# image-rs/deflate-rs

Hardware: AMD Instinct MI355X
Metric: MB/s raw input encoded (Compression::Default) + compressed size vs ref (higher is better)
Workload: dtype u8; 1 GPU; enwik8 = enwik8-like synthetic text (tests/datagen.py text_like; --enwik8 PATH takes the real file): 100000000 bytes per GPU, Compression::Default, stream-exact (P1); bytes_per_gpu=100000000, level=Compression::Default, parallelism=shard1

## Files before the change

deflate-rs_amd/csrc/deflate_kernels.hip:

```cpp
#include <hip/hip_runtime.h>
#include <stdint.h>

#include <type_traits>

#ifdef MI355_MATCH_STATS
__device__ unsigned long long g_mstats[16];
__device__ unsigned long long g_sstats[16];
#define MI355_STAT_DECL uint32_t stat_[8] = {0, 0, 0, 0, 0, 0, 0, 0};
#define MI355_STAT(i, v) stat_[i] += (v);
#define MI355_STAT_FLUSH(policy)                                                          \
    for (int i_ = 0; i_ < 8; i_++) atomicAdd(&g_mstats[i_], (unsigned long long)stat_[i_]); \
    atomicMax((policy).wgmax, stat_[0]);                                                  \
    if ((threadIdx.x & 63) == 0) {                                                        \
        unsigned long long t_ = wall_clock64();                                           \
        atomicMax((policy).wgend, t_);                                                    \
        atomicAdd((policy).wgsum, t_ - (policy).t0);                                      \
    }
#endif
#include "stages.h"

namespace mi355 {

struct GBytes {
    const uint8_t* d;
// ... 203 lines not shown
}
constexpr uint32_t LINKS_PAD = 64 * 8 * LG + 64;

#ifndef MI355_MATCH_TILE
#define MI355_MATCH_TILE 21504
#endif
constexpr uint32_t MT = MI355_MATCH_TILE;
#ifndef MI355_MATCH_THREADS
#define MI355_MATCH_THREADS 1024
#endif
constexpr uint32_t MTHREADS = MI355_MATCH_THREADS;
#ifndef MI355_MATCH_U
#define MI355_MATCH_U 2
#endif
#ifndef MI355_MATCH_R
#define MI355_MATCH_R 8
#endif
#ifndef MI355_EXT_ROUNDS
#define MI355_EXT_ROUNDS 100
#endif
#ifndef MI355_EXT_DENSE
#define MI355_EXT_DENSE 1
#endif
constexpr uint32_t MCHAINS = MI355_MATCH_U;
constexpr uint32_t MW_BYTES = WINDOW_SIZE + MT + 258 + 14;
constexpr uint32_t MW_LINKS = WINDOW_SIZE + MT;

struct MatchEmit {
    uint32_t* M;
    uint32_t* Mq;
    uint64_t wstart;
    __device__ void operator()(uint32_t idx, uint32_t m, uint32_t mq) const {
        M[wstart + idx] = m;
        if (Mq) Mq[wstart + idx] = mq;
    }
};

struct TileNext {
    uint32_t* counter;
    uint32_t base, count;
    __device__ uint32_t operator()() {
        uint32_t i = atomicAdd(counter, 1u);
        return i < count ? base + i : (uint32_t)NO_POS;
    }
};
struct WavePolicy {
#ifdef MI355_MATCH_STATS
    uint32_t* wgmax;
    unsigned long long* wgend;
    unsigned long long* wgsum;
    unsigned long long t0;
#endif
    __device__ bool operator()(bool pending, bool walking, uint32_t iter) const {
        if ((iter % MI355_MATCH_R) == MI355_MATCH_R - 1) return true;
        return __builtin_amdgcn_ballot_w64(walking) == 0;
    }
    __device__ bool keep_extending(bool any, uint32_t round) const {
        uint32_t cnt = (uint32_t)__popcll(__builtin_amdgcn_ballot_w64(any));
        return cnt >= MI355_EXT_DENSE || (round < MI355_EXT_ROUNDS && cnt > 0);
    }
};

struct TileLimit {
    SegEnds sg;
    uint64_t wstart;
    uint32_t one;
    __device__ uint32_t operator()(uint32_t idx) const {
        if (sg.m == 1) return one;
        uint64_t e = seg_end(sg, wstart + idx);
        uint64_t r = e - wstart;
        return r > 0xFFFFFFFFull ? 0xFFFFFFFFu : (uint32_t)r;
    }
};

template <bool HAS_Q>
__global__ __launch_bounds__(MTHREADS) void k_match(const uint8_t* __restrict__ in, uint32_t n,
                                                    const uint16_t* __restrict__ link, uint32_t* __restrict__ M,
                                                    uint32_t* __restrict__ Mq, uint32_t checks, uint32_t checks_q,
                                                    int in_aligned4, SegEnds sg, uint32_t mt) {
    __shared__ __attribute__((aligned(16))) uint8_t s_win[MW_BYTES + 2 * MW_LINKS];
    uint8_t* const s_bytes = s_win;
    uint16_t* const s_link = reinterpret_cast<uint16_t*>(s_win + MW_BYTES);
    __shared__ uint32_t s_next;
    const uint32_t tid = threadIdx.x;
    const uint64_t E = (uint64_t)blockIdx.x * mt;
    const uint32_t wbytes = WINDOW_SIZE + mt + 258 + 14, wlinks = WINDOW_SIZE + mt;
    const uint64_t wstart = E >= WINDOW_SIZE ? E - WINDOW_SIZE : 0;
    uint32_t* sb32 = reinterpret_cast<uint32_t*>(s_bytes);
    if (in_aligned4) {
        for (uint32_t w = tid; w < wbytes / 16; w += MTHREADS) {
            uint64_t g = wstart + 16ull * w;
            uint4 v = make_uint4(0, 0, 0, 0);
            if (g + 16 <= n) {
                v = *reinterpret_cast<const uint4*>(in + g);
            } else {
                uint32_t t[4] = {0, 0, 0, 0};
                for (int b = 0; b < 16; b++)
                    if (g + b < n) t[b >> 2] |= (uint32_t)in[g + b] << (8 * (b & 3));
                v = make_uint4(t[0], t[1], t[2], t[3]);
            }
            reinterpret_cast<uint4*>(s_bytes)[w] = v;
        }
    } else {
        for (uint32_t w = tid; w < wbytes / 4; w += MTHREADS) {
            uint64_t g = wstart + 4ull * w;
            uint32_t v = 0;
            for (int b = 0; b < 4; b++)
                if (g + b < n) v |= (uint32_t)in[g + b] << (8 * b);
            sb32[w] = v;
        }
    }
    for (uint32_t w = tid; w < wlinks / 8; w += MTHREADS) {
        uint64_t g = wstart + 8ull * w;
        uint4 v = make_uint4(0, 0, 0, 0);
        if (g + 8 <= n) {
            v = *reinterpret_cast<const uint4*>(link + g);
        } else {
            uint32_t t[4] = {0, 0, 0, 0};
            for (int b = 0; b < 8; b++)
                if (g + b < n) t[b >> 1] |= (uint32_t)link[g + b] << (16 * (b & 1));
            v = make_uint4(t[0], t[1], t[2], t[3]);
        }
        uint32_t t4[4] = {v.x, v.y, v.z, v.w};
#pragma unroll
        for (int q = 0; q < 4; q++) {
            uint32_t lo = t4[q] & 0xffffu, hi = t4[q] >> 16;
            t4[q] = (lo ? lo : 0xffffu) | ((hi ? hi : 0xffffu) << 16);
        }
        reinterpret_cast<uint4*>(s_link)[w] = make_uint4(t4[0], t4[1], t4[2], t4[3]);
    }
    if (tid == 0) s_next = 0;
#ifdef MI355_MATCH_STATS
    __shared__ uint32_t s_wgmax;
    __shared__ unsigned long long s_wgend, s_wgsum;
    if (tid == 0) {
        s_wgmax = 0;
        s_wgend = 0;
        s_wgsum = 0;
    }
    const unsigned long long t_enter = wall_clock64();
#endif
    __syncthreads();
    LdsWin win{s_bytes, s_link};
    MatchEmit emit{M, HAS_Q ? Mq : nullptr, wstart};
    TileNext next{&s_next, (uint32_t)(E - wstart), mt};
#ifdef MI355_MATCH_STATS
    const unsigned long long t_start = wall_clock64();
    WavePolicy pol{&s_wgmax, &s_wgend, &s_wgsum, t_start};
#else
    WavePolicy pol;
#endif
    TileLimit lim{sg, wstart, sg.m == 1 ? (uint32_t)(sg.ends[0] - wstart) : 0u};
    match_walk_park<MCHAINS, HAS_Q>(win, next, lim, checks, checks_q, emit, pol);
#ifdef MI355_MATCH_STATS
    __syncthreads();
    if (tid == 0) {
        atomicAdd(&g_mstats[8], (unsigned long long)s_wgmax);
        atomicAdd(&g_mstats[9], 1ull);
        atomicAdd(&g_mstats[10], s_wgend - t_start);
        atomicAdd(&g_mstats[11], s_wgsum);
        atomicAdd(&g_mstats[12], t_start - t_enter);
    }
#endif
}

constexpr uint32_t BSTRIDE = WINDOW_SIZE + 8;
constexpr uint32_t SORT_CHUNK = WINDOW_SIZE / 16;

__device__ __forceinline__ uint32_t epoch_active(uint32_t n, uint64_t E) {
    const uint64_t act = n >= 2 ? (uint64_t)n - 2 : 0;
    return act > E ? (uint32_t)((act - E) < (uint64_t)WINDOW_SIZE ? (act - E) : (uint64_t)WINDOW_SIZE) : 0u;
}

__device__ __forceinline__ uint32_t block_excl_scan_1024(uint32_t v, uint32_t* red , uint32_t* total) {
    const uint32_t lane = threadIdx.x & 63, wv = threadIdx.x >> 6;
    uint32_t x = v;
#pragma unroll
    for (int off = 1; off < 64; off <<= 1) {
        uint32_t y = __shfl_up(x, off, 64);
        if (lane >= (uint32_t)off) x += y;
    }
    __syncthreads();
    if (lane == 63) red[wv] = x;
    __syncthreads();
    uint32_t add = 0, all = 0;
#pragma unroll
    for (uint32_t k = 0; k < 16; k++) {
        const uint32_t t = red[k];
        add += k < wv ? t : 0u;
        all += t;
    }
    if (total) *total = all;
    return add + x - v;
}

template <int NB>
__device__ __forceinline__ void wave_match(uint32_t d, bool valid, uint32_t* plo, uint32_t* phi) {
    const uint64_t all = __builtin_amdgcn_ballot_w64(valid);
    uint32_t lo = (uint32_t)all, hi = (uint32_t)(all >> 32);
#pragma unroll
    for (int b = 0; b < NB; b++) {
        const int32_t mine = __builtin_amdgcn_sbfe((int32_t)d, (uint32_t)b, 1u);
        const uint64_t bal = __builtin_amdgcn_ballot_w64(mine != 0);
        lo &= ~((uint32_t)bal ^ (uint32_t)mine);
        hi &= ~((uint32_t)(bal >> 32) ^ (uint32_t)mine);
    }
    *plo = lo;
    *phi = hi;
}

#ifdef MI355_MATCH_STATS
#define KS_T(i)                                                                        \
    if (threadIdx.x == 0) {                                                            \
        unsigned long long t_ = __builtin_readcyclecounter();                          \
        atomicAdd(&g_sstats[i], t_ - ks_t);                                            \
        ks_t = t_;                                                                     \
    }
#else
#define KS_T(i)
#endif
template <int NB, class Dig, class Pay, class Put>
__device__ __forceinline__ void sort_pass(uint32_t J, uint32_t* cnt , uint32_t* red, Dig dig, Pay pay, Put put,
                                          unsigned long long& ks_t, int stat0) {
    constexpr uint32_t ND = 1u << NB;
    constexpr int NBAT = SORT_CHUNK / 64;
    const uint32_t tid = threadIdx.x, lane = tid & 63, wv = tid >> 6;
    uint32_t* mine = cnt + wv * 256;
    for (uint32_t k = lane; k < 256; k += 64) mine[k] = 0;
    wave_lds_fence();
    const uint32_t cb = wv * SORT_CHUNK;
    uint32_t dc[NBAT / 4];
    uint32_t bt[NBAT / 4];
    uint32_t Jc = J;
    asm volatile("" : "+s"(Jc));
#pragma unroll
    for (int b = 0; b < NBAT; b++) {
        const uint32_t i = cb + 64 * b + lane;
        const bool valid = i < Jc;
        const uint32_t d = valid ? dig(i) : 0u;
        uint32_t plo, phi;
        wave_match<NB>(d, valid, &plo, &phi);
        const uint32_t below = __builtin_amdgcn_mbcnt_hi(phi, __builtin_amdgcn_mbcnt_lo(plo, 0u));
        const uint32_t total = (uint32_t)__builtin_popcount(plo) + (uint32_t)__builtin_popcount(phi);
        if (valid && below == 0) atomicAdd(&mine[d], total);
        if ((b & 3) == 0)
            dc[b >> 2] = d;
        else
            dc[b >> 2] |= d << (8 * (b & 3));
        const uint32_t pk = below | (below + 1 == total ? 64u : 0u) | (valid ? 128u : 0u);
        if ((b & 3) == 0)
            bt[b >> 2] = pk;
        else
            bt[b >> 2] |= pk << (8 * (b & 3));
        if ((b & 3) == 3) __builtin_amdgcn_sched_barrier(0);
    }
    __syncthreads();
    KS_T(stat0)
    uint32_t v[4] = {0, 0, 0, 0}, sum = 0;
    const uint32_t d4 = tid >> 2, w4 = (tid & 3) * 4;
    if (d4 < ND) {
#pragma unroll
        for (int k = 0; k < 4; k++) {
            v[k] = cnt[(w4 + k) * 256 + d4];
            sum += v[k];
        }
    }
    uint32_t base = block_excl_scan_1024(sum, red, nullptr);
    if (d4 < ND) {
#pragma unroll
        for (int k = 0; k < 4; k++) {
            cnt[(w4 + k) * 256 + d4] = base;
            base += v[k];
        }
    }
    __syncthreads();
    KS_T(stat0 + 1)
#pragma unroll
    for (int b = 0; b < NBAT; b++) {
        const uint32_t i = cb + 64 * b + lane;
        const uint32_t d = (dc[b >> 2] >> (8 * (b & 3))) & 0xffu;
        const uint32_t pk = (bt[b >> 2] >> (8 * (b & 3))) & 0xffu;
        const bool valid = (pk & 128u) != 0;
        const uint32_t py = valid ? pay(i) : 0u;
        const uint32_t below = pk & 63u;
        uint32_t at = 0;
        if (valid) at = mine[d];
        wave_lds_fence();
        if (valid) {
            put(at + below, py);
            if (pk & 64u) mine[d] = at + below + 1;
        }
        wave_lds_fence();
    }
    __syncthreads();
    KS_T(stat0 + 2)
}

#ifndef MI355_SORT_HOT
#define MI355_SORT_HOT 4
#endif
#ifndef MI355_SORT_ROUNDS
#define MI355_SORT_ROUNDS 1
#endif
#ifndef MI355_SORT_SB
#define MI355_SORT_SB 4
#endif
template <int NB, bool LOW, class Dig, class Pay, class Put>
__device__ __forceinline__ void sort_pass_rtn(uint32_t J, uint32_t* cnt , uint32_t* red, Dig dig, Pay pay, Put put,
                                              unsigned long long& ks_t, int stat0, bool hot_low) {
    constexpr uint32_t ND = 1u << NB;
    constexpr int NBAT = SORT_CHUNK / 64;
    const uint32_t tid = threadIdx.x, lane = tid & 63, wv = tid >> 6;
    uint32_t* mine = cnt + wv * 256;
    for (uint32_t k = lane; k < 256; k += 64) mine[k] = 0;
    wave_lds_fence();
    const uint32_t cb = wv * SORT_CHUNK;
    uint32_t dc[NBAT / 4];
    uint32_t rk[NBAT / 2];
    uint32_t Jc = J;
    asm volatile("" : "+s"(Jc));
#pragma unroll
    for (int b = 0; b < NBAT; b++) {
        const uint32_t i = cb + 64 * b + lane;
        const bool valid = i < Jc;
        const uint32_t d = valid ? dig(i) : 0u;
        const uint64_t vm = __builtin_amdgcn_ballot_w64(valid);
        uint32_t r = 0;
        uint64_t left = vm;
        bool mine_done = !valid;
#pragma unroll
        for (int round = 0; round < MI355_SORT_ROUNDS; round++) {
            if (LOW && !hot_low) break;
            if (left == 0) break;
            const uint32_t first = (uint32_t)__builtin_ctzll(left);
            const uint32_t dk = (uint32_t)__builtin_amdgcn_readlane((int)d, (int)first);
            const uint64_t mk = __builtin_amdgcn_ballot_w64(!mine_done && d == dk);
            const uint32_t nk = (uint32_t)__popcll(mk);
            if (nk < MI355_SORT_HOT) break;
            const uint32_t at = mine[dk];
            wave_lds_fence();
            const bool hot = !mine_done && d == dk;
            if (hot) r = at + __builtin_amdgcn_mbcnt_hi((uint32_t)(mk >> 32), __builtin_amdgcn_mbcnt_lo((uint32_t)mk, 0u));
            if (lane == first) mine[dk] = at + nk;
            wave_lds_fence();
            mine_done = mine_done || hot;
            left &= ~mk;
        }
        if (!mine_done) r = atomicAdd(&mine[d], 1u);
        if ((b & 3) == 0)
            dc[b >> 2] = d;
        else
            dc[b >> 2] |= d << (8 * (b & 3));
        const uint32_t pk = r | (valid ? 0x8000u : 0u);
        if ((b & 1) == 0)
            rk[b >> 1] = pk;
        else
            rk[b >> 1] |= pk << 16;
        if ((b % MI355_SORT_SB) == MI355_SORT_SB - 1) __builtin_amdgcn_sched_barrier(0);
    }
    __syncthreads();
    KS_T(stat0)
    uint32_t v[4] = {0, 0, 0, 0}, sum = 0;
    const uint32_t d4 = tid >> 2, w4 = (tid & 3) * 4;
    if (d4 < ND) {
#pragma unroll
        for (int k = 0; k < 4; k++) {
            v[k] = cnt[(w4 + k) * 256 + d4];
            sum += v[k];
        }
    }
    uint32_t base = block_excl_scan_1024(sum, red, nullptr);
    if (d4 < ND) {
#pragma unroll
        for (int k = 0; k < 4; k++) {
            cnt[(w4 + k) * 256 + d4] = base;
            base += v[k];
        }
    }
    __syncthreads();
    KS_T(stat0 + 1)
#pragma unroll
    for (int b = 0; b < NBAT; b++) {
        const uint32_t i = cb + 64 * b + lane;
        const uint32_t d = (dc[b >> 2] >> (8 * (b & 3))) & 0xffu;
        const uint32_t pk = (rk[b >> 1] >> (16 * (b & 1))) & 0xffffu;
        if (pk & 0x8000u) put(mine[d] + (pk & 0x7fffu), pay(i));
    }
    __syncthreads();
    KS_T(stat0 + 2)
}

__global__ __launch_bounds__(1024) void k_lds_order_test(uint32_t rounds, uint32_t* bad) {
    __shared__ uint32_t sCnt[16 * 256];
    const uint32_t tid = threadIdx.x, lane = tid & 63, wv = tid >> 6;
    uint32_t* mine = sCnt + wv * 256;
    for (uint32_t k = lane; k < 256; k += 64) mine[k] = 0;
    __syncthreads();
    uint32_t x = (blockIdx.x * 1024 + tid) * 2654435761u + 12345u, wrong = 0;
    for (uint32_t r = 0; r < rounds; r++) {
        x = x * 1664525u + 1013904223u;
        const uint32_t kind = (r + wv) & 7u;
        const uint32_t mask = kind == 0 ? 0u : kind == 1 ? 1u : kind == 2 ? 3u : kind == 3 ? 7u : kind == 4 ? 15u : kind == 5 ? 63u : 255u;
        uint32_t d = (x >> 13) & mask;
        if (kind == 7) d = (lane >> 2) & 255u;
        const bool valid = ((x >> 5) & 15u) != 0 || kind < 2;
        uint32_t plo, phi;
        wave_match<8>(d, valid, &plo, &phi);
        const uint32_t below = __builtin_amdgcn_mbcnt_hi(phi, __builtin_amdgcn_mbcnt_lo(plo, 0u));
        uint32_t before = 0;
        if (valid) before = mine[d];
        wave_lds_fence();
        uint32_t got = 0;
        if (valid) got = atomicAdd(&mine[d], 1u);
        wave_lds_fence();
        if (valid && got != before + below) wrong++;
    }
    if (wrong) atomicAdd(bad, wrong);
}

#ifndef MI355_SWZ_BANKS
#define MI355_SWZ_BANKS 14
#endif
#ifndef MI355_SWZ_PERSISTENT
#define MI355_SWZ_PERSISTENT 0
#endif
#ifndef MI355_SORT_P1
#define MI355_SORT_P1 8
#endif
struct SortInit {
    uint32_t* sc;
    uint32_t sc_words;
    uint32_t* seg_end;
    uint32_t seg_val;
};
template <int MODE>
__device__ __forceinline__ void k_sort_body(uint32_t bx_, const uint8_t* in, uint32_t n, HashOverride ov,
                                               uint16_t* Sg, uint16_t* Bg, uint32_t e0, uint32_t dbl,
                                               SortInit init) {
    __shared__ __attribute__((aligned(16))) uint16_t sH[WINDOW_SIZE];
    __shared__ __attribute__((aligned(16))) uint32_t sBuf[WINDOW_SIZE / 2];
    __shared__ uint32_t sCnt[16 * 256];
    __shared__ uint32_t sRed[16];
    __shared__ uint32_t s_runs;
    const uint32_t tid = threadIdx.x;
    if (tid == 0) s_runs = 0;
    if (init.sc && bx_ == 0) {
        for (uint32_t i = tid; i < init.sc_words; i += 1024) init.sc[i] = 0;
        if (tid == 0 && init.seg_end) *init.seg_end = init.seg_val;
    }
    const uint32_t e = e0 + bx_;
    const uint64_t E = (uint64_t)e * WINDOW_SIZE;
    const uint32_t J = epoch_active(n, E);
    unsigned long long ks_t = __builtin_readcyclecounter();
    (void)ks_t;
    for (uint32_t k = tid; k < WINDOW_SIZE / 2; k += 1024) sBuf[k] = 0;
    __syncthreads();
    const bool whole = J == WINDOW_SIZE && (reinterpret_cast<uintptr_t>(in) & 15) == 0 && E + WINDOW_SIZE + 4 <= (uint64_t)n &&
                       !(ov.on | ov.m);
    if (whole) {
        uint2 wr[WINDOW_SIZE / (8 * 1024)];
        uint32_t nr[WINDOW_SIZE / (8 * 1024)];
#pragma unroll
        for (uint32_t r = 0; r < WINDOW_SIZE / (8 * 1024); r++) {
            const uint32_t i = (r * 1024 + tid) * 8;
            wr[r] = *reinterpret_cast<const uint2*>(in + E + i);
            nr[r] = *reinterpret_cast<const uint32_t*>(in + E + i + 8);
        }
#pragma unroll
        for (uint32_t r = 0; r < WINDOW_SIZE / (8 * 1024); r++) {
            const uint32_t i = (r * 1024 + tid) * 8;
            const uint2 w = wr[r];
            const uint32_t nx = nr[r];
            const uint32_t d[3] = {w.x, w.y, nx};
            uint32_t hs[8];
            const bool run1 = w.x == w.y && w.y == nx && w.x == __builtin_amdgcn_alignbyte(w.x, w.x, 1u);
            const uint32_t w0 = (uint32_t)__builtin_amdgcn_readfirstlane((int)w.x);
            const bool wave_run = __builtin_amdgcn_ballot_w64(!run1 || w.x != w0) == 0;
#pragma unroll
            for (int k = 0; k < 8; k++) {
                const uint32_t v = (k & 3) ? __builtin_amdgcn_alignbyte(d[(k >> 2) + 1], d[k >> 2], (uint32_t)(k & 3)) : d[k >> 2];
                hs[k] = hash3(v & 0xff, (v >> 8) & 0xff, (v >> 16) & 0xff);
                if (!wave_run) atomicAdd(&sBuf[hs[k] >> 1], (hs[k] & 1) ? 0x10000u : 1u);
            }
            *reinterpret_cast<uint4*>(&sH[i]) = make_uint4(hs[0] | (hs[1] << 16), hs[2] | (hs[3] << 16), hs[4] | (hs[5] << 16), hs[6] | (hs[7] << 16));
            if (wave_run && (tid & 63) == 0) {
                atomicAdd(&sBuf[hs[0] >> 1], (hs[0] & 1) ? 512u << 16 : 512u);
                atomicAdd(&s_runs, 1u);
            }
        }
    } else
    for (uint32_t i0 = 0; i0 < J; i0 += 8 * 1024) {
        uint32_t v[8];
#pragma unroll
        for (int k = 0; k < 8; k++) {
            const uint32_t i = i0 + 1024 * k + tid;
            const uint64_t p = E + (i < J ? i : 0u);
            if (n >= 4) {
                v[k] = load_u32_clamped(in, p, n);
            } else {
                v[k] = (uint32_t)in[p] | ((uint32_t)in[p + 1] << 8) | ((uint32_t)in[p + 2] << 16);
            }
        }
#pragma unroll
        for (int k = 0; k < 8; k++) {
            const uint32_t i = i0 + 1024 * k + tid;
            if (i < J) {
                const uint32_t ab = rewarm_ab(ov, E + i, v[k] & 0xff, (v[k] >> 8) & 0xff);
                const uint32_t h = hash3(ab & 0xff, ab >> 8, (v[k] >> 16) & 0xff);
                sH[i] = (uint16_t)h;
                atomicAdd(&sBuf[h >> 1], (h & 1) ? 0x10000u : 1u);
            }
        }
    }
    __syncthreads();
    KS_T(0)
    {
        uint32_t wds[16], sum = 0;
        const uint4* src = reinterpret_cast<const uint4*>(sBuf + tid * 16);
#pragma unroll
        for (int q = 0; q < 4; q++) {
            const uint4 x = src[q];
            wds[4 * q] = x.x;
            wds[4 * q + 1] = x.y;
            wds[4 * q + 2] = x.z;
            wds[4 * q + 3] = x.w;
        }
#pragma unroll
        for (int q = 0; q < 16; q++) sum += (wds[q] & 0xffffu) + (wds[q] >> 16);
        uint32_t run = block_excl_scan_1024(sum, sRed, nullptr);
        uint32_t outw[16];
#pragma unroll
        for (int q = 0; q < 16; q++) {
            const uint32_t lo = run;
            run += wds[q] & 0xffffu;
            const uint32_t hi = run;
            run += wds[q] >> 16;
            outw[q] = lo | (hi << 16);
        }
        if (tid == 1023) {
            Bg[(size_t)e * BSTRIDE + WINDOW_SIZE] = (uint16_t)J;
            Bg[(size_t)e * BSTRIDE + WINDOW_SIZE + 1] = s_runs > WINDOW_SIZE / 512 / 2 ? 1 : 0;
        }
        uint4* cur = reinterpret_cast<uint4*>(sBuf + tid * 16);
#pragma unroll
        for (int q = 0; q < 4; q++) cur[q] = make_uint4(outw[4 * q], outw[4 * q + 1], outw[4 * q + 2], outw[4 * q + 3]);
    }
    __syncthreads();
    {
        uint4* dst = reinterpret_cast<uint4*>(Bg + (size_t)e * BSTRIDE);
        const uint4* src = reinterpret_cast<const uint4*>(sBuf);
#pragma unroll
        for (uint32_t k = 0; k < WINDOW_SIZE / 8 / 1024; k++) dst[k * 1024 + tid] = src[k * 1024 + tid];
    }
    KS_T(1)
    uint16_t* buf16 = reinterpret_cast<uint16_t*>(sBuf);
    if (MODE == 1) {
        constexpr int P1 = MI355_SORT_P1;
        const bool runs_here = __builtin_amdgcn_readfirstlane((int)s_runs) != 0;
        sort_pass_rtn<P1, true>(
            J, sCnt, sRed, [&](uint32_t i) { return (uint32_t)sH[i] & ((1u << P1) - 1u); }, [&](uint32_t i) { return i; },
            [&](uint32_t at, uint32_t v) { buf16[at] = (uint16_t)v; }, ks_t, 2, runs_here);
        sort_pass_rtn<15 - P1, false>(
            J, sCnt, sRed, [&](uint32_t i) { return (uint32_t)sH[buf16[i]] >> P1; }, [&](uint32_t i) { return (uint32_t)buf16[i]; },
            [&](uint32_t at, uint32_t v) { sH[at] = (uint16_t)v; }, ks_t, 5, false);
    } else {
    sort_pass<8>(
        J, sCnt, sRed, [&](uint32_t i) { return (uint32_t)sH[i] & 255u; }, [&](uint32_t i) { return i; },
        [&](uint32_t at, uint32_t v) { buf16[at] = (uint16_t)v; }, ks_t, 2);
    sort_pass<7>(
        J, sCnt, sRed, [&](uint32_t i) { return (uint32_t)sH[buf16[i]] >> 8; }, [&](uint32_t i) { return (uint32_t)buf16[i]; },
        [&](uint32_t at, uint32_t v) { sH[at] = (uint16_t)v; }, ks_t, 5);
    }
#ifdef MI355_DEBUG_HOOKS
    if ((dbl & 2u) && tid == 0) {
        for (uint32_t i = 1; i < J; i++) {
            const uint32_t a = sH[i - 1], b = sH[i];
            const uint8_t* pa = in + E + a;
            const uint8_t* pb = in + E + b;
            if (E + b + 2 < n && hash3(pa[0], pa[1], pa[2]) == hash3(pb[0], pb[1], pb[2])) {
                sH[i - 1] = (uint16_t)b;
                sH[i] = (uint16_t)a;
                break;
            }
        }
    }
    __syncthreads();
    dbl &= 1u;
#endif
    if (MI355_SWZ_BANKS) {
        __syncthreads();
        if (tid < 8) sRed[tid] = 0;
        __syncthreads();
        if (tid < 256 && J >= 1024) {
            const uint32_t q = tid >> 6;
            const uint32_t bank = ((uint32_t)sH[(2 * q + 1) * (J / 8) + (tid & 63)] >> 1) & 63u;
            atomicOr(&sRed[2 * q + (bank >> 5)], 1u << (bank & 31));
        }
        __syncthreads();
        if (tid == 0) {
            uint32_t few = 0, very = 0;
            for (int q = 0; q < 4; q++) {
                const uint32_t nb = (uint32_t)(__popc(sRed[2 * q]) + __popc(sRed[2 * q + 1]));
                few += nb <= MI355_SWZ_BANKS ? 1u : 0u;
                very += nb <= MI355_SWZ_BANKS / 2 ? 1u : 0u;
            }
            Bg[(size_t)e * BSTRIDE + WINDOW_SIZE + 2] = (J >= 1024 && (few >= 2 || very >= 1) && dbl) ? 1 : 0;
        }
    }
    uint4* out = reinterpret_cast<uint4*>(Sg + (size_t)e * WINDOW_SIZE);
    const uint4* fin = reinterpret_cast<const uint4*>(sH);
    for (uint32_t k = tid; k < (J + 7) / 8; k += 1024) {
        const uint4 v = fin[k];
        out[k] = make_uint4(v.x << dbl, v.y << dbl, v.z << dbl, v.w << dbl);
    }
}
template <int MODE>
__global__ __launch_bounds__(1024) void k_sort(const uint8_t* __restrict__ in, uint32_t n, HashOverride ov,
                                               uint16_t* __restrict__ Sg, uint16_t* __restrict__ Bg, uint32_t e0, uint32_t dbl,
                                               SortInit init) {
    k_sort_body<MODE>(blockIdx.x, in, n, ov, Sg, Bg, e0, dbl, init);
}

#ifdef MI355_MATCH_STATS
#define M2_CNT(i, v) \
    if (((MI355_MATCH_STATS) & 2) || (i) == 0 || (i) == 4) m2c[i] += (uint32_t)(v);
#define M2_T0 uint32_t m2t = ((MI355_MATCH_STATS) & 1) ? (uint32_t)__builtin_readcyclecounter() : 0u;
#define M2_T(i)                                                      \
    if ((MI355_MATCH_STATS) & 1) {                                   \
        const uint32_t t_ = (uint32_t)__builtin_readcyclecounter();  \
        m2c[i] += t_ - m2t;                                          \
        m2t = t_;                                                    \
    }
#else
#define M2_CNT(i, v)
#define M2_T0
#define M2_T(i)
#endif

constexpr uint32_t M3T = 1024;
constexpr uint32_t M3_PAIRS = 2 * WINDOW_SIZE + 258 + 14;

template <bool SWZ>
struct PairWinT {
    const uint16_t* sb;
    uint32_t tbase;
    typedef __attribute__((address_space(3))) const uint16_t* lds_u16;
    enum : uint32_t { SH = 1 };
    __device__ uint32_t key_at(uint32_t a) const { return *(lds_u16)(SWZ ? m3_swz(a) : a); }
    __device__ void load16(uint32_t pos, uint32_t* q) const {
        typedef uint32_t u32x2 __attribute__((ext_vector_type(2)));
        u32x2 d0, d1, d2, d3, d4;
        const uint32_t a8 = (tbase + 2 * pos) & ~7u;
        if (SWZ) {
            asm volatile(
                "ds_read_b64 %0, %5\n\t"
                "ds_read_b64 %1, %6\n\t"
                "ds_read_b64 %2, %7\n\t"
                "ds_read_b64 %3, %8\n\t"
                "ds_read_b64 %4, %9\n\t"
                "s_waitcnt lgkmcnt(0)"
                : "=&v"(d0), "=&v"(d1), "=&v"(d2), "=&v"(d3), "=&v"(d4)
                : "v"(m3_swz(a8)), "v"(m3_swz(a8 + 8)), "v"(m3_swz(a8 + 16)), "v"(m3_swz(a8 + 24)), "v"(m3_swz(a8 + 32))
                : "memory");
        } else
        asm volatile(
            "ds_read_b64 %0, %5\n\t"
            "ds_read_b64 %1, %5 offset:8\n\t"
            "ds_read_b64 %2, %5 offset:16\n\t"
            "ds_read_b64 %3, %5 offset:24\n\t"
            "ds_read_b64 %4, %5 offset:32\n\t"
            "s_waitcnt lgkmcnt(0)"
            : "=&v"(d0), "=&v"(d1), "=&v"(d2), "=&v"(d3), "=&v"(d4)
            : "v"(a8)
            : "memory");
        const uint32_t w0 = __builtin_amdgcn_perm(d0.y, d0.x, 0x05040100u), w1 = __builtin_amdgcn_perm(d1.y, d1.x, 0x05040100u),
                       w2 = __builtin_amdgcn_perm(d2.y, d2.x, 0x05040100u), w3 = __builtin_amdgcn_perm(d3.y, d3.x, 0x05040100u),
                       w4 = __builtin_amdgcn_perm(d4.y, d4.x, 0x05040100u);
        q[0] = __builtin_amdgcn_alignbyte(w1, w0, pos);
        q[1] = __builtin_amdgcn_alignbyte(w2, w1, pos);
        q[2] = __builtin_amdgcn_alignbyte(w3, w2, pos);
        q[3] = __builtin_amdgcn_alignbyte(w4, w3, pos);
    }
    __device__ uint32_t load32(uint32_t pos) const {
        if (SWZ) return key_at(tbase + 2 * pos) | (key_at(tbase + 2 * pos + 4) << 16);
        lds_u16 t = (lds_u16)(tbase + 2 * pos);
        return (uint32_t)t[0] | ((uint32_t)t[2] << 16);
    }
    __device__ uint32_t sidx(uint32_t i) const { return sb[(int64_t)(int32_t)i]; }
};
typedef PairWinT<false> PairWin;

struct MsGroup {
    uint32_t t0, t1, t2, t3, t4, t5, t6, t7, a0, a1, a2, a3, a4, a5, a6, a7, probe;
};
__device__ __forceinline__ void ms_decode(const MsGroup st, uint64_t* any_out, uint32_t* asel_out, uint32_t* back_out) {
    uint32_t asel_o = st.a0, back_o = 0;
#define MS_STEP(T, A, OFF)                 \
    {                                      \
        const bool h_ = st.T == st.probe;  \
        asel_o = h_ ? st.A : asel_o;          \
        back_o = h_ ? OFF : back_o;          \
    }
    MS_STEP(t7, a7, 2u) MS_STEP(t6, a6, 4u) MS_STEP(t5, a5, 6u) MS_STEP(t4, a4, 8u)
    MS_STEP(t3, a3, 10u) MS_STEP(t2, a2, 12u) MS_STEP(t1, a1, 14u) MS_STEP(t0, a0, 16u)
#undef MS_STEP
    *any_out = __builtin_amdgcn_ballot_w64(back_o != 0);
    *asel_out = asel_o;
    *back_out = back_o ? back_o : 16u;
}

#define MF_ADD(F, A, REG, HALF) \
    "v_add_u32_sdwa %[" F A "], " REG ", %[" F "bb] dst_sel:DWORD dst_unused:UNUSED_PAD src0_sel:" HALF " src1_sel:DWORD\n\t"
#ifndef MI355_STEP_WAITS
#define MI355_STEP_WAITS 2
#endif
#define MF_CMPW(F, N, T) "s_waitcnt lgkmcnt(" N ")\n\tv_cmpx_ne_u32_e32 vcc, %[" F T "], %[" F "probe]\n\t"
#define MF_CMPN(F, N, T) "v_cmpx_ne_u32_e32 vcc, %[" F T "], %[" F "probe]\n\t"
#define MF_CMP(F, N, T) MF_CMPW(F, N, T)
#define MF_ADDS8(F, R0, R1, R2, R3)                                                                                  \
    MF_ADD(F, "a0", R3, "WORD_1") MF_ADD(F, "a1", R3, "WORD_0") MF_ADD(F, "a2", R2, "WORD_1") MF_ADD(F, "a3", R2, "WORD_0") \
    MF_ADD(F, "a4", R1, "WORD_1") MF_ADD(F, "a5", R1, "WORD_0") MF_ADD(F, "a6", R0, "WORD_1") MF_ADD(F, "a7", R0, "WORD_0")
#define MF_RD8_0(F)                                                                                                  \
    "ds_read_u16 %[" F "t0], %[" F "a0]\n\tds_read_u16 %[" F "t1], %[" F "a1]\n\tds_read_u16 %[" F "t2], %[" F "a2]\n\t"    \
    "ds_read_u16 %[" F "t3], %[" F "a3]\n\tds_read_u16 %[" F "t4], %[" F "a4]\n\tds_read_u16 %[" F "t5], %[" F "a5]\n\t"    \
    "ds_read_u16 %[" F "t6], %[" F "a6]\n\tds_read_u16 %[" F "t7], %[" F "a7]\n\t"
#define MF_SW1(F, T, A)                                                                                   \
    "v_lshrrev_b32_e32 %[" F T "], 5, %[" F A "]\n\tv_and_b32_e32 %[" F T "], 0xf8, %[" F T "]\n\t"       \
    "v_xor_b32_e32 %[" F T "], %[" F A "], %[" F T "]\n\tds_read_u16 %[" F T "], %[" F T "]\n\t"
#define MF_RD8_1(F)                                                                                           \
    MF_SW1(F, "t0", "a0") MF_SW1(F, "t1", "a1") MF_SW1(F, "t2", "a2") MF_SW1(F, "t3", "a3") MF_SW1(F, "t4", "a4") \
    MF_SW1(F, "t5", "a5") MF_SW1(F, "t6", "a6") MF_SW1(F, "t7", "a7")
#define MF_ISSUE8X(RD8, F, R0, R1, R2, R3) MF_ADDS8(F, R0, R1, R2, R3) RD8(F) "v_add_u32_e32 %[" F "offb], -16, %[" F "offb]\n\t"
#if MI355_STEP_WAITS == 8
#define MF_TEST8(F, N7, N6, N5, N4, N3, N2, N1, N0)                                                               \
    MF_CMP(F, N7, "t0") MF_CMP(F, N6, "t1") MF_CMP(F, N5, "t2") MF_CMP(F, N4, "t3")                                \
    MF_CMP(F, N3, "t4") MF_CMP(F, N2, "t5") MF_CMP(F, N1, "t6") MF_CMP(F, N0, "t7")                                \
    "v_cmpx_ge_u32_e32 vcc, %[" F "a7], %[" F "lowa]\n\t"                                                         \
    "v_cmpx_ge_i32_e32 vcc, %[" F "offb], %[" F "endb]\n\t"
#elif MI355_STEP_WAITS == 4
#define MF_TEST8(F, N7, N6, N5, N4, N3, N2, N1, N0)                                                               \
    MF_CMPW(F, N6, "t0") MF_CMPN(F, N6, "t1") MF_CMPW(F, N4, "t2") MF_CMPN(F, N4, "t3")                            \
    MF_CMPW(F, N2, "t4") MF_CMPN(F, N2, "t5") MF_CMPW(F, N0, "t6") MF_CMPN(F, N0, "t7")                            \
    "v_cmpx_ge_u32_e32 vcc, %[" F "a7], %[" F "lowa]\n\t"                                                         \
    "v_cmpx_ge_i32_e32 vcc, %[" F "offb], %[" F "endb]\n\t"
#elif MI355_STEP_WAITS == 2
#define MF_TEST8(F, N7, N6, N5, N4, N3, N2, N1, N0)                                                               \
    MF_CMPW(F, N4, "t0") MF_CMPN(F, N4, "t1") MF_CMPN(F, N4, "t2") MF_CMPN(F, N4, "t3")                            \
    MF_CMPW(F, N0, "t4") MF_CMPN(F, N0, "t5") MF_CMPN(F, N0, "t6") MF_CMPN(F, N0, "t7")                            \
    "v_cmpx_ge_u32_e32 vcc, %[" F "a7], %[" F "lowa]\n\t"                                                         \
    "v_cmpx_ge_i32_e32 vcc, %[" F "offb], %[" F "endb]\n\t"
#else
#define MF_TEST8(F, N7, N6, N5, N4, N3, N2, N1, N0)                                                               \
    MF_CMPW(F, N0, "t0") MF_CMPN(F, N0, "t1") MF_CMPN(F, N0, "t2") MF_CMPN(F, N0, "t3")                            \
    MF_CMPN(F, N0, "t4") MF_CMPN(F, N0, "t5") MF_CMPN(F, N0, "t6") MF_CMPN(F, N0, "t7")                            \
    "v_cmpx_ge_u32_e32 vcc, %[" F "a7], %[" F "lowa]\n\t"                                                         \
    "v_cmpx_ge_i32_e32 vcc, %[" F "offb], %[" F "endb]\n\t"
#endif
#define MF_OPS(F, S)                                                                                                        \
    [F##offb] "+v"(S.offb), [F##a0] "=&v"(S.a0), [F##a1] "=&v"(S.a1), [F##a2] "=&v"(S.a2), [F##a3] "=&v"(S.a3), [F##a4] "=&v"(S.a4), \
    [F##a5] "=&v"(S.a5), [F##a6] "=&v"(S.a6), [F##a7] "=&v"(S.a7), [F##t0] "=&v"(S.t0), [F##t1] "=&v"(S.t1), [F##t2] "=&v"(S.t2), \
    [F##t3] "=&v"(S.t3), [F##t4] "=&v"(S.t4), [F##t5] "=&v"(S.t5), [F##t6] "=&v"(S.t6), [F##t7] "=&v"(S.t7)
#define MF_INS(F, S) [F##bb] "v"(S.bb2), [F##lowa] "v"(S.lowa2), [F##probe] "v"(S.probe), [F##endb] "v"(S.endb)

#define MF_ONE(RD8, F, W, C, RA, RB, R0, R1, R2, R3, R4, R5, R6, R7)                           \
        "s_mov_b64 exec, %[" W "]\n\t"                                                      \
        "global_load_dwordx4 " RA ", %[" F "offb], %[sb] offset:-14\n\t"                    \
        "global_load_dwordx4 " RB ", %[" F "offb], %[sb] offset:-30\n\t"                    \
        "s_waitcnt vmcnt(1)\n\t"                                                            \
        MF_ISSUE8X(RD8, F, R0, R1, R2, R3)                                                        \
        MF_TEST8(F, "7", "6", "5", "4", "3", "2", "1", "0")                                 \
        "s_cbranch_execz .Lmf_one" F "%=\n\t"                                               \
        "s_waitcnt vmcnt(0)\n\t"                                                            \
        MF_ISSUE8X(RD8, F, R4, R5, R6, R7)                                                        \
        MF_TEST8(F, "7", "6", "5", "4", "3", "2", "1", "0")                                 \
        ".Lmf_one" F "%=:\n\t"                                                              \
        "s_mov_b64 %[" C "], exec\n\t"

#define MS_STEPS_DUAL_DEF(NAME, RD8) \
template <bool HAS_Q> \
__device__ __forceinline__ void NAME(SwG<HAS_Q>& x, SwG<HAS_Q>& y, const uint16_t* sb8, uint64_t walkx, uint64_t walky, \
                                              uint64_t* stillx, uint64_t* stilly) { \
    uint64_t save, cx, cy; \
    asm volatile( \
        "s_mov_b64 %[save], exec\n\t" \
 \
 \
 \
        "s_mov_b64 %[cx], 0\n\t" \
        "s_mov_b64 %[cy], 0\n\t" \
        "s_cmp_eq_u64 %[wy], 0\n\t" \
        "s_cbranch_scc1 .Lmf_xonly%=\n\t" \
        "s_cmp_eq_u64 %[wx], 0\n\t" \
        "s_cbranch_scc1 .Lmf_yonly%=\n\t" \
        "s_mov_b64 exec, %[wx]\n\t" \
        "global_load_dwordx4 v[56:59], %[xoffb], %[sb] offset:-14\n\t" \
        "global_load_dwordx4 v[60:63], %[xoffb], %[sb] offset:-30\n\t" \
        "s_mov_b64 exec, %[wy]\n\t" \
        "global_load_dwordx4 v[64:67], %[yoffb], %[sb] offset:-14\n\t" \
        "global_load_dwordx4 v[68:71], %[yoffb], %[sb] offset:-30\n\t" \
        "s_mov_b64 exec, %[wx]\n\t" \
        "s_waitcnt vmcnt(3)\n\t" \
        MF_ISSUE8X(RD8, "x", "v56", "v57", "v58", "v59") \
        "s_mov_b64 exec, %[wy]\n\t" \
        "s_waitcnt vmcnt(1)\n\t" \
        MF_ISSUE8X(RD8, "y", "v64", "v65", "v66", "v67") \
        "s_mov_b64 exec, %[wx]\n\t" \
        MF_TEST8("x", "15", "14", "13", "12", "11", "10", "9", "8") \
        "s_mov_b64 %[cx], exec\n\t" \
        "s_mov_b64 exec, %[wy]\n\t" \
        MF_TEST8("y", "7", "6", "5", "4", "3", "2", "1", "0") \
        "s_mov_b64 %[cy], exec\n\t" \
        "s_or_b64 vcc, %[cx], %[cy]\n\t" \
        "s_cbranch_scc0 .Lmf_end%=\n\t" \
        "s_waitcnt vmcnt(0)\n\t" \
        "s_mov_b64 exec, %[cx]\n\t" \
        MF_ISSUE8X(RD8, "x", "v60", "v61", "v62", "v63") \
        "s_mov_b64 exec, %[cy]\n\t" \
        MF_ISSUE8X(RD8, "y", "v68", "v69", "v70", "v71") \
        "s_mov_b64 exec, %[cx]\n\t" \
        MF_TEST8("x", "15", "14", "13", "12", "11", "10", "9", "8") \
        "s_mov_b64 %[cx], exec\n\t" \
        "s_mov_b64 exec, %[cy]\n\t" \
        MF_TEST8("y", "7", "6", "5", "4", "3", "2", "1", "0") \
        "s_mov_b64 %[cy], exec\n\t" \
        "s_branch .Lmf_end%=\n\t" \
        ".Lmf_xonly%=:\n\t" \
        MF_ONE(RD8, "x", "wx", "cx", "v[56:59]", "v[60:63]", "v56", "v57", "v58", "v59", "v60", "v61", "v62", "v63") \
        "s_branch .Lmf_end%=\n\t" \
        ".Lmf_yonly%=:\n\t" \
        MF_ONE(RD8, "y", "wy", "cy", "v[64:67]", "v[68:71]", "v64", "v65", "v66", "v67", "v68", "v69", "v70", "v71") \
        ".Lmf_end%=:\n\t" \
        "s_waitcnt vmcnt(0)\n\t" \
        "s_mov_b64 exec, %[save]\n\t" \
        : MF_OPS(x, x), MF_OPS(y, y), [save] "=&s"(save), [cx] "=&s"(cx), [cy] "=&s"(cy) \
        : MF_INS(x, x), MF_INS(y, y), [sb] "s"(sb8), [wx] "s"(walkx), [wy] "s"(walky) \
        : "vcc", "scc", "memory", "v56", "v57", "v58", "v59", "v60", "v61", "v62", "v63", "v64", "v65", "v66", "v67", "v68", "v69", \
          "v70", "v71"); \
    *stillx = cx; \
    *stilly = cy; \
}
MS_STEPS_DUAL_DEF(ms_steps_dual, MF_RD8_0)
MS_STEPS_DUAL_DEF(ms_steps_dual_swz, MF_RD8_1)
#undef MF_ONE

constexpr uint32_t ADV_TILE = 1024, ADV_HALO = 260;
struct TileM {
    const uint32_t* t;
    __device__ uint32_t operator()(uint32_t r) const { return t[r]; }
};
__device__ __forceinline__ uint32_t rel_end(const SegEnds& sg, uint64_t base, uint32_t r) {
    const uint64_t e = (uint64_t)seg_end(sg, base + r) - base;
    return e > 0xFFFFFFFFull ? 0xFFFFFFFFu : (uint32_t)e;
}
template <bool HAS_Q, bool SWZ, bool SINGLE = false>
__device__ __forceinline__ void m3_epoch(uint4* s_T, uint32_t& s_next, const uint32_t e, const uint32_t part, const uint8_t* __restrict__ in, uint32_t n,
                                         const uint16_t* __restrict__ Sg, const uint16_t* __restrict__ Bg, uint32_t* __restrict__ M,
                                         uint32_t* __restrict__ Mq, uint32_t checks, uint32_t checks_q, int in_aligned16, SegEnds sg,
                                         HashOverride ov, uint32_t split, uint32_t* __restrict__ Ms, uint32_t* __restrict__ Mqs,
                                         uint32_t* __restrict__ sort_bad) {
    constexpr uint32_t pair = SINGLE ? 1u : 2u;
    const uint32_t tid = threadIdx.x, lane = tid & 63;
#ifdef MI355_MATCH_STATS
    uint32_t m2c[16] = {0, 0, 0, 0, 0, 0, 0, 0, 0, 0, 0, 0, 0, 0, 0, 0};
#endif
    M2_T0
    const uint64_t E = (uint64_t)e * WINDOW_SIZE;
    const uint64_t wbase = e ? E - WINDOW_SIZE : 0;
// ... 1969 lines not shown
```

Before: 23490 MB/s.

## Merge hot-digit aggregation with atomic ranking and specialize full-window sort

```diff
diff --git a/deflate-rs_amd/csrc/deflate_kernels.hip b/deflate-rs_amd/csrc/deflate_kernels.hip
--- a/deflate-rs_amd/csrc/deflate_kernels.hip
+++ b/deflate-rs_amd/csrc/deflate_kernels.hip
@@ -529,10 +529,25 @@
 #ifndef MI355_SORT_ROUNDS
 #define MI355_SORT_ROUNDS 1
 #endif
+#ifndef MI355_SORT_MERGE
+#define MI355_SORT_MERGE 1
+#endif
+#ifndef MI355_SORT_NEIGH
+#define MI355_SORT_NEIGH 1
+#endif
+#ifndef MI355_SORT_TWO
+#define MI355_SORT_TWO 0
+#endif
+#ifndef MI355_SORT_HOT2
+#define MI355_SORT_HOT2 1
+#endif
+#ifndef MI355_SORT_WHOLE
+#define MI355_SORT_WHOLE 1
+#endif
 #ifndef MI355_SORT_SB
 #define MI355_SORT_SB 4
 #endif
-template <int NB, bool LOW, class Dig, class Pay, class Put>
+template <int NB, bool LOW, bool WHOLE, class Dig, class Pay, class Put>
 __device__ __forceinline__ void sort_pass_rtn(uint32_t J, uint32_t* cnt , uint32_t* red, Dig dig, Pay pay, Put put,
                                               unsigned long long& ks_t, int stat0, bool hot_low) {
     constexpr uint32_t ND = 1u << NB;
@@ -549,17 +564,50 @@
 #pragma unroll
     for (int b = 0; b < NBAT; b++) {
         const uint32_t i = cb + 64 * b + lane;
-        const bool valid = i < Jc;
+        const bool valid = WHOLE || i < Jc;
         const uint32_t d = valid ? dig(i) : 0u;
         const uint64_t vm = __builtin_amdgcn_ballot_w64(valid);
         uint32_t r = 0;
         uint64_t left = vm;
         bool mine_done = !valid;
+        uint64_t eqm = 0;
+        if (MI355_SORT_NEIGH && !LOW) {
+            const uint32_t prev = (uint32_t)__builtin_amdgcn_update_dpp(-1, (int)d, 0x138 , 0xf, 0xf, false);
+            eqm = __builtin_amdgcn_ballot_w64(valid && d == prev);
+        }
+        if (MI355_SORT_MERGE && !LOW) {
+            constexpr uint64_t TOP = 1ull << 63;
+            const uint32_t f1 = (uint32_t)__builtin_ctzll((eqm ? eqm : vm) | TOP);
+            const uint32_t d1 = (uint32_t)__builtin_amdgcn_readlane((int)d, (int)f1);
+            const uint64_t m1 = __builtin_amdgcn_ballot_w64(valid && d == d1);
+            const uint32_t n1 = (uint32_t)__popcll(m1);
+            const bool in1 = n1 >= MI355_SORT_HOT2 && valid && d == d1;
+            uint32_t f2 = 0, n2 = 0;
+            uint64_t m2 = 0;
+            bool in2 = false;
+            if (MI355_SORT_TWO) {
+                const uint64_t rest = vm & ~m1, eq2 = eqm & ~m1;
+                f2 = (uint32_t)__builtin_ctzll((eq2 ? eq2 : rest) | TOP);
+                const uint32_t d2 = (uint32_t)__builtin_amdgcn_readlane((int)d, (int)f2);
+                m2 = __builtin_amdgcn_ballot_w64(valid && d == d2 && d != d1);
+                n2 = (uint32_t)__popcll(m2);
+                in2 = n2 >= MI355_SORT_HOT2 && valid && d == d2 && d != d1;
+            }
+            const uint32_t add = in1 ? n1 : in2 ? n2 : 1u;
+            if (valid && ((!in1 && !in2) || (in1 && lane == f1) || (in2 && lane == f2))) r = atomicAdd(&mine[d], add);
+            const uint32_t at1 = (uint32_t)__builtin_amdgcn_readlane((int)r, (int)f1);
+            if (in1) r = at1 + __builtin_amdgcn_mbcnt_hi((uint32_t)(m1 >> 32), __builtin_amdgcn_mbcnt_lo((uint32_t)m1, 0u));
+            if (MI355_SORT_TWO) {
+                const uint32_t at2 = (uint32_t)__builtin_amdgcn_readlane((int)r, (int)f2);
+                if (in2) r = at2 + __builtin_amdgcn_mbcnt_hi((uint32_t)(m2 >> 32), __builtin_amdgcn_mbcnt_lo((uint32_t)m2, 0u));
+            }
+            mine_done = true;
+        } else {
 #pragma unroll
         for (int round = 0; round < MI355_SORT_ROUNDS; round++) {
             if (LOW && !hot_low) break;
             if (left == 0) break;
-            const uint32_t first = (uint32_t)__builtin_ctzll(left);
+            const uint32_t first = (uint32_t)__builtin_ctzll((eqm & left) ? (eqm & left) : left);
             const uint32_t dk = (uint32_t)__builtin_amdgcn_readlane((int)d, (int)first);
             const uint64_t mk = __builtin_amdgcn_ballot_w64(!mine_done && d == dk);
             const uint32_t nk = (uint32_t)__popcll(mk);
@@ -573,6 +621,7 @@
             mine_done = mine_done || hot;
             left &= ~mk;
         }
+        }
         if (!mine_done) r = atomicAdd(&mine[d], 1u);
         if ((b & 3) == 0)
             dc[b >> 2] = d;
@@ -611,7 +660,7 @@
         const uint32_t i = cb + 64 * b + lane;
         const uint32_t d = (dc[b >> 2] >> (8 * (b & 3))) & 0xffu;
         const uint32_t pk = (rk[b >> 1] >> (16 * (b & 1))) & 0xffffu;
-        if (pk & 0x8000u) put(mine[d] + (pk & 0x7fffu), pay(i));
+        if (WHOLE || (pk & 0x8000u)) put(mine[d] + (pk & 0x7fffu), pay(i));
     }
     __syncthreads();
     KS_T(stat0 + 2)
@@ -784,12 +833,19 @@
     if (MODE == 1) {
         constexpr int P1 = MI355_SORT_P1;
         const bool runs_here = __builtin_amdgcn_readfirstlane((int)s_runs) != 0;
-        sort_pass_rtn<P1, true>(
-            J, sCnt, sRed, [&](uint32_t i) { return (uint32_t)sH[i] & ((1u << P1) - 1u); }, [&](uint32_t i) { return i; },
-            [&](uint32_t at, uint32_t v) { buf16[at] = (uint16_t)v; }, ks_t, 2, runs_here);
-        sort_pass_rtn<15 - P1, false>(
-            J, sCnt, sRed, [&](uint32_t i) { return (uint32_t)sH[buf16[i]] >> P1; }, [&](uint32_t i) { return (uint32_t)buf16[i]; },
-            [&](uint32_t at, uint32_t v) { sH[at] = (uint16_t)v; }, ks_t, 5, false);
+        auto dig1 = [&](uint32_t i) { return (uint32_t)sH[i] & ((1u << P1) - 1u); };
+        auto pay1 = [&](uint32_t i) { return i; };
+        auto put1 = [&](uint32_t at, uint32_t v) { buf16[at] = (uint16_t)v; };
+        auto dig2 = [&](uint32_t i) { return (uint32_t)sH[buf16[i]] >> P1; };
+        auto pay2 = [&](uint32_t i) { return (uint32_t)buf16[i]; };
+        auto put2 = [&](uint32_t at, uint32_t v) { sH[at] = (uint16_t)v; };
+        if (MI355_SORT_WHOLE && J == WINDOW_SIZE) {
+            sort_pass_rtn<P1, true, true>(J, sCnt, sRed, dig1, pay1, put1, ks_t, 2, runs_here);
+            sort_pass_rtn<15 - P1, false, true>(J, sCnt, sRed, dig2, pay2, put2, ks_t, 5, false);
+        } else {
+            sort_pass_rtn<P1, true, false>(J, sCnt, sRed, dig1, pay1, put1, ks_t, 2, runs_here);
+            sort_pass_rtn<15 - P1, false, false>(J, sCnt, sRed, dig2, pay2, put2, ks_t, 5, false);
+        }
     } else {
     sort_pass<8>(
         J, sCnt, sRed, [&](uint32_t i) { return (uint32_t)sH[i] & 255u; }, [&](uint32_t i) { return i; },
```

Measured after the change: 23630 MB/s (median of 6 runs). About the same (+0.6%).
